# ldyken53/gaussian-splatting-wgpu

Hardware: AMD Instinct MI355X
Metric: frames/sec (higher is better)
Workload: dtype f32; 1 GPU; bicycle-like synthetic 6.1M gaussians @1920x1080; gaussians=6100000, width=1920, height=1080, tile_size=16, parallelism=single GPU, visible=2430918, processed=15909895, block_evaluated=6068168, sort_passes=1, depth_ordered_emission=True, tight_binning=True, blend_mode=fused, camera=64-step orbit, moved every frame

## Files before the change

### gaussian-splatting-wgpu_amd/csrc/gs_kernels.h

```cpp
#pragma once
#include "gs_device.h"

void gs_launch_repack(const void* d_aos, uint32_t n, const GsScene& s, hipStream_t st);
void gs_launch_ply_chunk(const void* d_raw, uint32_t m, uint32_t first, const GsPlyTable& t, const GsScene& s, hipStream_t st);
struct GsPreprocessLaunch {
    const void* func;
    uint32_t blocks;
    GsScene s; GsUniforms u; GsFrame f;
    void* gdata; uint32_t* counts; GsTightOut to;
    void* args[6];
};
void gs_preprocess_prepare(GsPreprocessLaunch& L, const GsScene& s, const GsUniforms& u, const GsFrame& f, void* gdata, uint32_t* counts,
                           bool tight, uint32_t* arena, uint32_t* rowptr, GsControl* ctl, uint32_t tight_nb = 0);
void gs_launch_preprocess(GsPreprocessLaunch& L, hipStream_t st);
void gs_launch_zero(void* p, uint64_t bytes, hipStream_t st);
uint32_t gs_scan_blocks(uint32_t n);
void gs_launch_scan(const uint32_t* counts, uint32_t n, uint32_t* offsets, unsigned long long* status, uint32_t* ticket, GsControl* ctl,
                    hipStream_t st);
uint64_t gs_emit_chunks(uint64_t capacity);
void gs_launch_emit_balanced(const void* gdata, const void* grec, const uint32_t* chunk_table, const GsFrame& f, uint32_t* keys, uint32_t* values,
                             GsControl* ctl, uint32_t grid, uint32_t hist_bits, uint32_t hist_passes, bool keys16, hipStream_t st);
void gs_launch_emit(const void* gdata, const uint32_t* counts, const uint32_t* offsets, const uint32_t* perm, const uint32_t* n_dev,
                    const GsFrame& f, uint32_t* keys, uint32_t* values, GsControl* ctl, hipStream_t st);
void gs_launch_ranges16(const uint16_t* tiles, const GsControl* ctl, uint32_t capacity, uint32_t T, uint32_t* ranges, uint32_t grid,
                        uint32_t* sticky, GsReport* rep, hipStream_t st);
void gs_launch_rebuild_keys(const uint16_t* tiles, const uint32_t* vals, const uint32_t* counts, uint32_t count, uint32_t n, uint32_t id_mask,
                            uint32_t* keys, hipStream_t st);
void gs_launch_ranges(const uint32_t* keys, const GsControl* ctl, uint32_t capacity, uint32_t T, uint32_t* ranges, uint32_t grid,
                      uint32_t* sticky, GsReport* rep, hipStream_t st);
uint32_t gs_sort_tiles(uint64_t capacity);
void gs_launch_sort(uint32_t* keysA, uint32_t* valsA, uint32_t* keysB, uint32_t* valsB, GsControl* ctl, uint32_t* tickets, uint32_t* hist,
                    const uint32_t* n_ptr, uint32_t capacity, uint32_t passes, uint32_t bits, uint32_t by_tile, uint32_t* status,
                    uint32_t grid, bool have_hist, const uint32_t* aux_table, uint32_t* aux_out, hipStream_t st, uint32_t** out_keys,
                    uint32_t** out_vals, bool keys16 = false);
int gs_launch_blend(const void* gdata, const uint32_t* values, const uint32_t* ranges, const GsFrame& f, uint32_t* rgba8, float* rgbf,
                    bool aux, float* alpha, float* depth, GsControl* ctl, uint32_t* tile_depth, bool exact, uint32_t ablation, bool masked, hipStream_t st, uint32_t* prof = nullptr,
                    uint32_t* prof_blocks = nullptr);
void gs_launch_debug_view(const uint32_t* ranges, const GsFrame& f, uint32_t view, uint32_t* rgba8, hipStream_t st);
void gs_launch_assemble(const void* slabs, void* image, uint32_t width, uint32_t height, const uint32_t* d_px_bounds, uint32_t n_slabs,
                        uint64_t slab_stride_px, hipStream_t st);
uint32_t gs_gsort_tiles(uint32_t n);
uint64_t gs_gsort_scratch_bytes(uint32_t n);
void gs_launch_gsort(const uint32_t* words, const uint32_t* aux_in, uint32_t n, void* scratch, void* grec, uint32_t* chunk_table, uint32_t chunk_cap,
                     uint32_t* tot_visible, uint32_t* tot_quantity, hipStream_t st);
uint32_t gs_rows_sort_tiles(uint64_t row_cap);
uint32_t gs_rows_chunks(uint64_t row_cap);
void gs_launch_rows(const uint32_t* arena, const void* grec, const uint32_t* chunk_table, uint32_t* rows_sorted, GsControl* ctl, uint32_t* sort_status, uint32_t row_cap,
                    uint32_t* M3, uint32_t* tileoff, uint32_t* rowtot, const GsFrame& f, uint32_t* values, uint32_t* ranges, uint32_t cus,
                    uint32_t* sticky, GsReport* rep, hipStream_t st, void (*mark)(void*, int), void* mark_arg);
void gs_launch_rows_rebuild_keys(const uint32_t* ranges, uint32_t T, const uint32_t* vals, const uint32_t* counts, uint32_t count, uint32_t n,
                                 uint32_t* keys, hipStream_t st);
void gs_launch_pick(const void* gdata, const uint32_t* values, const uint32_t* ranges, const GsFrame& f, uint32_t id_mask, const void* d_queries,
                    uint32_t n, void* d_results, uint32_t max_contrib, void* d_contrib, hipStream_t st);
```

### gaussian-splatting-wgpu_amd/csrc/gs_runtime.hip

```cpp
#include <hip/hip_runtime.h>

#include <algorithm>
#include <cmath>
#include <cstdarg>
#include <cstddef>
#include <cstdio>
#include <cstring>
#include <mutex>
#include <new>
#include <vector>

#include "../../include/gsplat/gs_abi.h"
#include "gs_kernels.h"
#include "gs_tight.h"

#define GS_EXPORT extern "C" __attribute__((visibility("default")))

static thread_local char g_err[512] = "";
static int32_t fail(int32_t code, const char* fmt, ...) {
    va_list ap;
    va_start(ap, fmt);
    vsnprintf(g_err, sizeof(g_err), fmt, ap);
    va_end(ap);
    return code;
// ... 336 lines not shown
    if (n) gs_launch_repack(d_aos, (uint32_t)n, c->scene, c->stream);
    HIP_TRY(hipGetLastError());
    HIP_TRY(hipStreamSynchronize(c->stream));
    return GS_OK;
}

static int32_t drop_shadows(gs_ctx* c) {
    for (gs_ctx* s : c->shadows) gs_destroy(s);
    c->shadows.clear();
    c->last = c;
    c->rr = 0;
    c->cap_hint = 0;
    c->row_hint = 0;
    return GS_OK;
}
GS_EXPORT int32_t gs_share_splats(gs_ctx* c, gs_ctx* owner) {
    if (!c || !owner || c == owner) return fail(GS_ERR_INVALID_ARGUMENT, "gs_share_splats: needs two distinct contexts");
    if (c->cfg.device != owner->cfg.device) return fail(GS_ERR_INVALID_ARGUMENT, "gs_share_splats: contexts are on different devices");
    if (!c->is_shadow) drop_shadows(c);
    if (!owner->scene_mem) return fail(GS_ERR_NO_SCENE, "gs_share_splats: the owner holds no splats");
    HIP_TRY(hipSetDevice(c->cfg.device));
    if (c->pending) { int32_t rc = wait_one(c); if (rc != GS_OK) return rc; }
    int32_t rc = alloc_per_gaussian(c, owner->n, c->cfg.max_intersections ? 0 : owner->capacity, owner->row_cap);
    if (rc != GS_OK) return rc;
    c->scene_mem = owner->scene_mem;
    c->scene_bytes = owner->scene_bytes;
    c->scene = owner->scene;
    c->scene_borrowed = true;
    HIP_TRY(hipStreamSynchronize(c->stream));
    return GS_OK;
}

GS_EXPORT int32_t gs_upload_splats_device(gs_ctx* c, const void* d_aos, uint64_t n) {
    if (!c || (!d_aos && n)) return fail(GS_ERR_INVALID_ARGUMENT, "gs_upload_splats_device: null argument");
    if (n >= (1ull << 31)) return fail(GS_ERR_INVALID_ARGUMENT, "gs_upload_splats: too many gaussians");
    HIP_TRY(hipSetDevice(c->cfg.device));
    drop_shadows(c);
    return upload_common(c, d_aos, n);
}

GS_EXPORT int32_t gs_upload_splats(gs_ctx* c, const void* aos, uint64_t n) {
    if (!c || (!aos && n)) return fail(GS_ERR_INVALID_ARGUMENT, "gs_upload_splats: null argument");
    if (n >= (1ull << 31)) return fail(GS_ERR_INVALID_ARGUMENT, "gs_upload_splats: too many gaussians");
    HIP_TRY(hipSetDevice(c->cfg.device));
    drop_shadows(c);
    void* d = nullptr;
    const size_t bytes = (size_t)n * GS_SPLAT_RECORD_BYTES;
    HIP_TRY(hipMalloc(&d, std::max<size_t>(bytes, 256)));
    if (bytes) {
        hipError_t e = hipMemcpy(d, aos, bytes, hipMemcpyHostToDevice);
        if (e != hipSuccess) { hipFree(d); return fail(GS_ERR_HIP, "upload memcpy: %s", hipGetErrorString(e)); }
    }
    int32_t rc = upload_common(c, d, n);
    hipFree(d);
    return rc;
}

static inline void mark(gs_ctx* c, int i) {
    if (!c->have_events) return;
    hipEventRecord(c->ev[c->frames % GS_EV_RING][i], c->stream);
    Roctx& r = roctx();
    if (r.push) {
        if (i > 0) r.pop();
        if (i < GS_STAGE_COUNT) r.push(kStageRange[i]);
    }
}

static void mark_cb(void* p, int i) { mark((gs_ctx*)p, i); }

static int32_t record_frame(gs_ctx* c, const GsUniforms& u, bool debug, void* ext_rgba8, bool tight) {
    const GsFrame& f = c->frame;
    hipStream_t st = c->stream;
    gs_launch_zero(c->ctl_mem, tight ? c->ctl_bytes_tight : c->ctl_bytes, st);
    c->h_ctl_valid = false;
    if (debug) HIP_TRY(hipMemsetAsync(c->gdata, 0, std::max<size_t>((size_t)c->n * 64, 256), st));
    mark(c, 0);
    gs_preprocess_prepare(c->pre, c->scene, u, f, c->gdata, c->counts, tight, c->arena, c->rowptr, c->ctl, c->tight_nb);
    gs_launch_preprocess(c->pre, st);
    mark(c, 1);
    const bool by_index = !tight && (debug || c->index_order);
    bool keys16 = false;
    if (tight) {
        gs_launch_gsort(c->counts, c->rowptr, c->n, c->gsort_scratch, c->grec, c->chunk_table, (uint32_t)gs_emit_chunks(std::max(c->capacity, c->row_cap)),
                        &c->ctl->num_visible, &c->ctl->num_slots, st);
        mark(c, 2);
        gs_launch_rows(c->arena, c->grec, c->chunk_table, c->rows_sorted, c->ctl, c->rows_status, (uint32_t)c->row_cap, c->M3, c->tileoff, c->rowtot, f, c->valsA,
                       c->ranges, c->grid_persist / 4u, c->sticky, c->h_rep, st, mark_cb, c);
        c->keysS = nullptr;
        c->valsS = c->valsA;
        mark(c, 4);
    } else if (by_index) {
        gs_launch_scan(c->counts, c->n, c->offsets, c->scan_status, &c->ctl->scan_ticket[0], c->ctl, st);
        mark(c, 2);
        gs_launch_emit(c->gdata, c->counts, c->offsets, nullptr, nullptr, f, c->keysA, c->valsA, c->ctl, st);
    } else {
        gs_launch_gsort(c->counts, nullptr, c->n, c->gsort_scratch, c->grec, c->chunk_table, (uint32_t)gs_emit_chunks(std::max(c->capacity, c->row_cap)),
                        &c->ctl->num_visible, &c->ctl->num_intersections, st);
        mark(c, 2);
        gs_launch_emit_balanced(c->gdata, c->grec, c->chunk_table, f, c->keysA, c->valsA, c->ctl, c->grid_persist * 2,
                                c->tile_bits, c->tile_passes, c->tile16, st);
        keys16 = c->tile16;
    }
    if (debug) {
        if (!c->keysU) {
            HIP_TRY(hipMalloc((void**)&c->keysU, (size_t)c->capacity * 4));
            HIP_TRY(hipMalloc((void**)&c->valsU, (size_t)c->capacity * 4));
        }
        HIP_TRY(hipMemcpyAsync(c->keysU, c->keysA, (size_t)c->capacity * 4, hipMemcpyDeviceToDevice, st));
        HIP_TRY(hipMemcpyAsync(c->valsU, c->valsA, (size_t)c->capacity * 4, hipMemcpyDeviceToDevice, st));
    }
    if (!tight) {
        mark(c, 3);
        if (by_index)
            gs_launch_sort(c->keysA, c->valsA, c->keysB, c->valsB, c->ctl, c->ctl->sort_ticket, &c->ctl->hist[0][0], &c->ctl->num_intersections,
                           (uint32_t)c->capacity, c->passes, 8, 0, c->sort_status, c->grid_persist, false, nullptr, nullptr, st, &c->keysS, &c->valsS);
        else
            gs_launch_sort(c->keysA, c->valsA, c->keysB, c->valsB, c->ctl, c->ctl->sort_ticket, &c->ctl->hist[0][0], &c->ctl->num_intersections,
                           (uint32_t)c->capacity, c->tile_passes, c->tile_bits, keys16 ? 0 : 1, c->sort_status, c->grid_persist, true,
                           nullptr, nullptr, st, &c->keysS, &c->valsS, keys16);
        mark(c, 4);
        if (keys16) gs_launch_ranges16((const uint16_t*)c->keysS, c->ctl, (uint32_t)c->capacity, c->T, c->ranges, c->grid_persist * 2, c->sticky, c->h_rep, st);
        else gs_launch_ranges(c->keysS, c->ctl, (uint32_t)c->capacity, c->T, c->ranges, c->grid_persist * 2, c->sticky, c->h_rep, st);
    }
    c->last_passes = tight ? 1u : (by_index ? c->passes : c->tile_passes);
    c->last_by_index = by_index;
    c->last_keys16 = keys16;
    c->last_tight = tight;
    mark(c, 5);
    uint32_t* target = ext_rgba8 ? (uint32_t*)ext_rgba8 : c->rgba8;
    if ((c->blend_ablation & 0x10000u) && !c->blend_prof) HIP_TRY(hipMalloc((void**)&c->blend_prof, (size_t)(1u << 20) * 16));
    const bool aux = (c->cfg.flags & GS_FLAG_AUX_OUTPUTS) != 0;
    const int walkers = gs_launch_blend(c->gdata, c->valsS, c->ranges, f, target, c->rgbf, aux, c->alpha, c->depth, c->ctl, c->tile_depth,
                                        (c->cfg.flags & GS_FLAG_EXACT_BLEND) != 0, c->blend_ablation & 0xFFFFu, tight, st,
                                        (c->blend_ablation & 0x10000u) ? c->blend_prof : nullptr, &c->blend_prof_blocks);
    if (walkers == -2) return fail(GS_ERR_INVALID_ARGUMENT, "blend: GS_FLAG_AUX_OUTPUTS without its alpha / depth planes");
    if (walkers < 0) return fail(GS_ERR_INVALID_ARGUMENT, "unsupported tile size %u", f.tile_size);
    c->blend_walkers = (uint32_t)walkers;
    mark(c, 6);
    if (c->debug_view) gs_launch_debug_view(c->ranges, f, c->debug_view, target, st);
    return GS_OK;
}

static void drop_graph(gs_ctx* c) {
    if (c->gexec) hipGraphExecDestroy(c->gexec);
    if (c->graph) hipGraphDestroy(c->graph);
    c->gexec = nullptr; c->graph = nullptr; c->pre_node = nullptr;
    c->graph_valid = false;
}

static int32_t enqueue_frame(gs_ctx* c, const GsUniforms& u, bool debug, void* ext_rgba8) {
    hipStream_t st = c->stream;
    if (c->emit_order == 2) {
        const uint64_t saved = c->passes > c->tile_passes ? c->passes - c->tile_passes : 0;
        c->index_order = !(c->have_frame && saved * (uint64_t)c->h_rep->num_intersections >= 1000000ull);
    } else {
        c->index_order = (c->emit_order == 1);
    }
    const bool tight = !debug && c->tile_cull && c->tight_ok && c->n < (1u << GS_ID_BITS);
    const bool graphable = c->use_graph && !debug && !c->have_events && !(c->blend_ablation & 0x10000u) && c->n;
    if (graphable) {
        if (!c->gexec || !c->graph_valid || c->gkey_index != c->index_order || c->gkey_tight != tight || c->gkey_ext != ext_rgba8 ||
            c->gkey_alpha != c->alpha || c->gkey_depth != c->depth) {
            if (c->gexec) HIP_TRY(hipStreamSynchronize(st));
            drop_graph(c);
            HIP_TRY(hipStreamBeginCapture(st, hipStreamCaptureModeRelaxed));
            const int32_t rc = record_frame(c, u, debug, ext_rgba8, tight);
            hipGraph_t g = nullptr;
            const hipError_t e = hipStreamEndCapture(st, &g);
            if (rc != GS_OK) { if (g) hipGraphDestroy(g); return rc; }
            if (e != hipSuccess || !g) return fail(GS_ERR_HIP, "frame graph capture: %s", hipGetErrorString(e));
            c->graph = g;
            HIP_TRY(hipGraphInstantiate(&c->gexec, g, nullptr, nullptr, 0));
            size_t nn = 0;
            HIP_TRY(hipGraphGetNodes(g, nullptr, &nn));
            std::vector<hipGraphNode_t> nodes(nn);
            HIP_TRY(hipGraphGetNodes(g, nodes.data(), &nn));
            uint32_t found = 0;
            for (hipGraphNode_t nd : nodes) {
                hipGraphNodeType ty;
                if (hipGraphNodeGetType(nd, &ty) != hipSuccess || ty != hipGraphNodeTypeKernel) continue;
// ... 796 lines not shown
```

### gaussian-splatting-wgpu_amd/csrc/k_gsort.hip

```cpp
#include "gs_device.h"

#define GC_ITEMS 8
#define GC_THREADS 256
#define GC (GC_THREADS * GC_ITEMS)
#define GBINS 1024
#define GS_EMIT_CHUNK_SHIFT 10
__device__ __forceinline__ uint64_t m_index(uint32_t b, uint32_t chunk, uint32_t NT) { return ((uint64_t)(b >> 3) * NT + chunk) * 8u + (b & 7u); }

__device__ __forceinline__ uint32_t sat32(unsigned long long v) { return v > 0xFFFFFFFFull ? 0xFFFFFFFFu : (uint32_t)v; }

__global__ __launch_bounds__(GC_THREADS) void gs_gsort_hist_kernel(const uint32_t* __restrict__ words, uint32_t n, uint2* __restrict__ M, uint32_t NT) {
    __shared__ uint32_t s_cnt[GBINS];
    __shared__ unsigned long long s_sum[GBINS];
    const uint32_t chunk = blockIdx.x, tid = threadIdx.x;
    for (uint32_t b = tid; b < GBINS; b += GC_THREADS) { s_cnt[b] = 0u; s_sum[b] = 0ull; }
    __syncthreads();
#pragma unroll
    for (int j = 0; j < GC_ITEMS; ++j) {
        const uint32_t k = chunk * GC + j * GC_THREADS + tid;
        if (k < n) {
            const uint32_t w = words[k];
            if (w & GS_COUNT_MASK) {
                const uint32_t b = w >> GS_COUNT_BITS;
                atomicAdd(&s_cnt[b], 1u);
                atomicAdd(&s_sum[b], (unsigned long long)(w & GS_COUNT_MASK));
            }
        }
    }
    __syncthreads();
#pragma unroll
    for (uint32_t i = 0; i < GBINS / GC_THREADS; ++i) {
        const uint32_t b = tid * (GBINS / GC_THREADS) + i;
        M[m_index(b, chunk, NT)] = make_uint2(s_cnt[b], sat32(s_sum[b]));
    }
}

struct GsPair { uint32_t x; unsigned long long y; };
__device__ __forceinline__ unsigned long long wave_incl_scan64(unsigned long long v, uint32_t lane) {
#pragma unroll
    for (int d = 1; d < 64; d <<= 1) {
        const uint32_t lo = __shfl_up((uint32_t)v, d, 64), hi = __shfl_up((uint32_t)(v >> 32), d, 64);
        if ((int)lane >= d) v += ((unsigned long long)hi << 32) | lo;
    }
    return v;
}
__device__ __forceinline__ GsPair block_excl2(GsPair v, uint32_t tid, GsPair* s_w , GsPair& total) {
    const uint32_t lane = tid & 63, w = tid >> 6;
    const uint32_t ix = wave_incl_scan(v.x, lane);
    const unsigned long long iy = wave_incl_scan64(v.y, lane);
    if (lane == 63) { s_w[w].x = ix; s_w[w].y = iy; }
    __syncthreads();
    GsPair base; base.x = 0u; base.y = 0ull;
    total.x = 0u; total.y = 0ull;
#pragma unroll
    for (int k = 0; k < GC_THREADS / 64; ++k) {
        const GsPair t = s_w[k];
        if (k < (int)w) { base.x += t.x; base.y += t.y; }
        total.x += t.x; total.y += t.y;
    }
    __syncthreads();
    GsPair r; r.x = base.x + ix - v.x; r.y = base.y + iy - v.y;
    return r;
}

#define GR_THREADS 1024
__device__ __forceinline__ void scan_stride8(uint32_t& x, unsigned long long& y, uint32_t lane) {
#pragma unroll
    for (int d = 8; d < 64; d <<= 1) {
        const uint32_t ox = __shfl_up(x, d, 64), lo = __shfl_up((uint32_t)y, d, 64), hi = __shfl_up((uint32_t)(y >> 32), d, 64);
        if ((int)lane >= d) { x += ox; y += ((unsigned long long)hi << 32) | lo; }
    }
}
__global__ __launch_bounds__(GR_THREADS) void gs_gsort_rowscan_kernel(uint2* __restrict__ M, uint32_t NT, uint32_t n, uint2* __restrict__ rowtot) {
    __shared__ uint32_t s_x[GR_THREADS / 64][8];
    __shared__ unsigned long long s_y[GR_THREADS / 64][8];
    const uint32_t nt = (n + GC - 1) / GC, tid = threadIdx.x, lane = tid & 63, w = tid >> 6, cl = tid >> 3, sub = tid & 7u;
    const uint32_t per = (nt + GR_THREADS / 8 - 1u) / (GR_THREADS / 8);
    const uint32_t c0 = cl * per < nt ? cl * per : nt, c1 = (cl + 1u) * per < nt ? (cl + 1u) * per : nt;
    uint2* row = M + (uint64_t)blockIdx.x * NT * 8u + sub;
    uint32_t ax = 0;
    unsigned long long ay = 0;
    for (uint32_t c = c0; c < c1; c += 8u) {
        uint2 v[8];
#pragma unroll
        for (int k = 0; k < 8; ++k) v[k] = (c + k < c1) ? row[(uint64_t)(c + k) * 8u] : make_uint2(0u, 0u);
#pragma unroll
        for (int k = 0; k < 8; ++k) { ax += v[k].x; ay += v[k].y; }
    }
    uint32_t ix = ax;
    unsigned long long iy = ay;
    scan_stride8(ix, iy, lane);
    if (lane >= 56u) { s_x[w][sub] = ix; s_y[w][sub] = iy; }
    __syncthreads();
    uint32_t rx = ix - ax, tx = 0;
    unsigned long long ry = iy - ay, ty = 0;
#pragma unroll
    for (uint32_t k = 0; k < GR_THREADS / 64; ++k) {
        const uint32_t vx = s_x[k][sub];
        const unsigned long long vy = s_y[k][sub];
        if (k < w) { rx += vx; ry += vy; }
        tx += vx; ty += vy;
    }
    for (uint32_t c = c0; c < c1; c += 8u) {
        uint2 v[8];
#pragma unroll
        for (int k = 0; k < 8; ++k) v[k] = (c + k < c1) ? row[(uint64_t)(c + k) * 8u] : make_uint2(0u, 0u);
#pragma unroll
        for (int k = 0; k < 8; ++k) {
            if (c + k < c1) row[(uint64_t)(c + k) * 8u] = make_uint2(rx, sat32(ry));
            rx += v[k].x; ry += v[k].y;
        }
    }
    if (tid < 8u) rowtot[blockIdx.x * 8u + sub] = make_uint2(tx, sat32(ty));
}

struct GsortShared {
    uint2 base[GBINS];
    unsigned short binstart[GBINS];
    union {
        unsigned short whist[GC_THREADS / 64][GBINS];
        uint32_t P[GC];
    } u;
    unsigned short id[GC];
    uint32_t word[GC], aux[GC];
    GsPair w2[GC_THREADS / 64];
    uint32_t wcnt[GC_THREADS / 64];
};
static_assert(sizeof(unsigned short) * (GC_THREADS / 64) * GBINS == sizeof(uint32_t) * GC, "the ranking counters and the prefix share their storage");

__global__ __launch_bounds__(GC_THREADS) void gs_gsort_scatter_kernel(const uint32_t* __restrict__ words, const uint32_t* __restrict__ aux_in, uint32_t n,
                                                                      const uint2* __restrict__ M, uint32_t NT, const uint2* __restrict__ rowtot,
                                                                      uint4* __restrict__ grec, uint32_t* __restrict__ chunk_table,
                                                                      uint32_t chunk_cap, uint32_t* __restrict__ tot_visible,
                                                                      uint32_t* __restrict__ tot_quantity) {
    __shared__ GsortShared S;
    const uint32_t chunk = blockIdx.x;
    const uint32_t tid = threadIdx.x, lane = tid & 63, w = tid >> 6;
    const unsigned long long lt_mask = (1ull << lane) - 1ull;
    constexpr uint32_t BPT = GBINS / GC_THREADS;

    uint32_t wv[GC_ITEMS], av[GC_ITEMS];
    const uint32_t e0 = chunk * GC + w * (64 * GC_ITEMS) + lane;
#pragma unroll
    for (int j = 0; j < GC_ITEMS; ++j) {
        const uint32_t k = e0 + j * 64;
        wv[j] = (k < n) ? words[k] : 0u;
        av[j] = (aux_in && k < n) ? aux_in[k] : 0u;
    }
    uint2 t[BPT], mm[BPT];
#pragma unroll
    for (uint32_t i = 0; i < BPT; ++i) { t[i] = rowtot[tid * BPT + i]; mm[i] = M[m_index(tid * BPT + i, chunk, NT)]; }

    {
        GsPair acc; acc.x = 0u; acc.y = 0ull;
#pragma unroll
        for (uint32_t i = 0; i < BPT; ++i) { acc.x += t[i].x; acc.y += t[i].y; }
        GsPair total;
        GsPair run = block_excl2(acc, tid, S.w2, total);
#pragma unroll
        for (uint32_t i = 0; i < BPT; ++i) {
            S.base[tid * BPT + i] = make_uint2(run.x + mm[i].x, sat32(run.y + mm[i].y));
            run.x += t[i].x; run.y += t[i].y;
        }
        if (chunk == 0 && tid == 0) { *tot_visible = total.x; *tot_quantity = sat32(total.y); }
    }
    for (uint32_t k = lane; k < GBINS; k += 64) S.u.whist[w][k] = 0;

    uint32_t wave_vis = 0;
#pragma unroll
    for (int j = 0; j < GC_ITEMS; ++j) {
        if (!(wv[j] & GS_COUNT_MASK)) wv[j] = 0u;
        wave_vis += (uint32_t)__popcll(__ballot(wv[j] != 0u));
    }
    if (lane == 0) S.wcnt[w] = wave_vis;
    __syncthreads();
    uint32_t cbase = 0, nc = 0;
#pragma unroll
    for (int k = 0; k < GC_THREADS / 64; ++k) { if (k < (int)w) cbase += S.wcnt[k]; nc += S.wcnt[k]; }
#pragma unroll
    for (int j = 0; j < GC_ITEMS; ++j) {
        const unsigned long long bal = __ballot(wv[j] != 0u);
        if (wv[j]) {
            const uint32_t p = cbase + (uint32_t)__popcll(bal & lt_mask);
            S.id[p] = (unsigned short)(w * (64 * GC_ITEMS) + j * 64 + lane);
            S.word[p] = wv[j];
            S.aux[p] = av[j];
        }
        cbase += (uint32_t)__popcll(bal);
    }
    for (uint32_t p = nc + tid; p < GC; p += GC_THREADS) S.word[p] = 0xFFFFFFFFu;
    __syncthreads();
    if (nc == 0) return;

    const uint32_t T = (nc + GC_THREADS - 1) / GC_THREADS;
    const uint32_t Q = T * 64;
    uint32_t gid[GC_ITEMS], wd[GC_ITEMS], ax[GC_ITEMS];
    uint32_t rank2[GC_ITEMS / 2];
#pragma unroll
    for (int j = 0; j < GC_ITEMS; ++j) {
        const uint32_t p = w * Q + j * 64 + lane;
        const bool in = (uint32_t)j < T;
        gid[j] = in ? (uint32_t)S.id[p] : 0u;
        wd[j] = in ? S.word[p] : 0xFFFFFFFFu;
        ax[j] = in ? S.aux[p] : 0u;
    }
#pragma unroll
    for (int j = 0; j < GC_ITEMS; ++j) {
        if ((uint32_t)j < T) {
            const uint32_t d = wd[j] >> GS_COUNT_BITS;
            uint32_t plo = 0xFFFFFFFFu, phi = 0xFFFFFFFFu;
#pragma unroll
            for (int b = 0; b < 10; ++b) {
                const uint32_t bit = (d >> b) & 1u;
                const unsigned long long bal = __ballot(bit != 0u);
                const uint32_t inv = bit - 1u;
                plo &= (uint32_t)bal ^ inv;
                phi &= (uint32_t)(bal >> 32) ^ inv;
            }
            const uint32_t below = __popc(plo & (uint32_t)lt_mask) + __popc(phi & (uint32_t)(lt_mask >> 32));
            const uint32_t cnt = __popc(plo) + __popc(phi);
            const uint32_t pre = S.u.whist[w][d];
            __builtin_amdgcn_fence(__ATOMIC_RELEASE, "wavefront");
            if (below == 0) S.u.whist[w][d] = (unsigned short)(pre + cnt);
            __builtin_amdgcn_fence(__ATOMIC_ACQUIRE, "wavefront");
            const uint32_t r = pre + below;
            if (j & 1) rank2[j >> 1] |= r << 16;
            else rank2[j >> 1] = r;
        }
    }
    __syncthreads();
    {
        uint32_t tot[BPT], acc = 0;
#pragma unroll
        for (uint32_t i = 0; i < BPT; ++i) {
            const uint32_t b = tid * BPT + i;
            uint32_t run = 0;
#pragma unroll
            for (int k = 0; k < GC_THREADS / 64; ++k) { const uint32_t c = S.u.whist[k][b]; S.u.whist[k][b] = (unsigned short)run; run += c; }
            tot[i] = run;
            acc += run;
        }
        GsPair total, in;
        in.x = acc; in.y = 0ull;
        const GsPair ex = block_excl2(in, tid, S.w2, total);
        uint32_t run = ex.x;
#pragma unroll
        for (uint32_t i = 0; i < BPT; ++i) { S.binstart[tid * BPT + i] = (unsigned short)run; run += tot[i]; }
    }
    __syncthreads();
    uint32_t mypos[GC_ITEMS];
#pragma unroll
    for (int j = 0; j < GC_ITEMS; ++j) {
        mypos[j] = 0xFFFFFFFFu;
        if ((uint32_t)j < T) {
            const uint32_t d = wd[j] >> GS_COUNT_BITS;
            const uint32_t r = (j & 1) ? (rank2[j >> 1] >> 16) : (rank2[j >> 1] & 0xFFFFu);
            mypos[j] = (uint32_t)S.binstart[d] + (uint32_t)S.u.whist[w][d] + r;
        }
    }
    __syncthreads();
#pragma unroll
    for (int j = 0; j < GC_ITEMS; ++j) {
        if ((uint32_t)j < T) {
            S.id[mypos[j]] = (unsigned short)gid[j];
            S.word[mypos[j]] = wd[j];
            S.aux[mypos[j]] = ax[j];
        }
    }
    __syncthreads();
    {
        uint32_t c[GC_ITEMS];
        unsigned long long acc = 0;
#pragma unroll
        for (int j = 0; j < GC_ITEMS; ++j) {
            const uint32_t p = tid * GC_ITEMS + j;
            const uint32_t x = (p < T * GC_THREADS) ? S.word[p] : 0xFFFFFFFFu;
            c[j] = x == 0xFFFFFFFFu ? 0u : (x & GS_COUNT_MASK);
            acc += c[j];
        }
        GsPair total, in;
        in.x = 0u; in.y = acc;
        const GsPair ex = block_excl2(in, tid, S.w2, total);
        unsigned long long run = ex.y;
#pragma unroll
        for (int j = 0; j < GC_ITEMS; ++j) { S.u.P[tid * GC_ITEMS + j] = sat32(run); run += c[j]; }
    }
    __syncthreads();
#pragma unroll
    for (int j = 0; j < GC_ITEMS; ++j) {
        const uint32_t pos = j * GC_THREADS + tid;
        if (pos >= nc) continue;
        const uint32_t x = S.word[pos];
        const uint32_t b = x >> GS_COUNT_BITS, first = S.binstart[b];
        const uint2 base = S.base[b];
        const uint32_t g = base.x + (pos - first);
        const unsigned long long off64 = (unsigned long long)base.y + (S.u.P[pos] - S.u.P[first]);
        const uint32_t off = sat32(off64);
        grec[g] = make_uint4(chunk * GC + (uint32_t)S.id[pos], x, off, S.aux[pos]);
        const uint32_t cnt = x & GS_COUNT_MASK;
        if (off != 0xFFFFFFFFu) {
            const unsigned long long lastq = (off64 + cnt - 1ull) >> GS_EMIT_CHUNK_SHIFT;
            const uint32_t last = lastq > 0xFFFFFFFFull ? 0xFFFFFFFFu : (uint32_t)lastq;
            for (uint32_t c = (uint32_t)((off64 + (1u << GS_EMIT_CHUNK_SHIFT) - 1ull) >> GS_EMIT_CHUNK_SHIFT); c <= last && c < chunk_cap; ++c) chunk_table[c] = g;
        }
    }
}

uint32_t gs_gsort_tiles(uint32_t n) { return (n + GC - 1) / GC; }
uint64_t gs_gsort_scratch_bytes(uint32_t n) { return ((uint64_t)GBINS * gs_gsort_tiles(n ? n : 1) + GBINS) * sizeof(uint2); }
void gs_launch_gsort(const uint32_t* words, const uint32_t* aux_in, uint32_t n, void* scratch, void* grec, uint32_t* chunk_table, uint32_t chunk_cap,
                     uint32_t* tot_visible, uint32_t* tot_quantity, hipStream_t st) {
    if (!n) return;
    const uint32_t NT = gs_gsort_tiles(n);
    uint2* M = (uint2*)scratch;
    uint2* rowtot = M + (uint64_t)GBINS * NT;
    hipLaunchKernelGGL(gs_gsort_hist_kernel, dim3(NT), dim3(GC_THREADS), 0, st, words, n, M, NT);
    hipLaunchKernelGGL(gs_gsort_rowscan_kernel, dim3(GBINS / 8), dim3(GR_THREADS), 0, st, M, NT, n, rowtot);
    hipLaunchKernelGGL(gs_gsort_scatter_kernel, dim3(NT), dim3(GC_THREADS), 0, st, words, aux_in, n, (const uint2*)M, NT, (const uint2*)rowtot,
                       (uint4*)grec, chunk_table, chunk_cap, tot_visible, tot_quantity);
}
```

Before: 1296 frames/s.

## Process multiple chunks per workgroup in gaussian depth sort with running bin bases

The histogram and scatter kernels of the gaussian depth-bin sort now each handle a run of consecutive chunks sized from the persistent grid, instead of one workgroup per chunk. Per-bin bases are carried forward across chunks inside the workgroup, and the next chunk's words are prefetched while the current one is processed. The histogram matrix shrinks to one column per run, which lightens the row scan. The scatter path also drops the separate compaction pass and ranks visible entries directly with ballots. The cost is less parallelism per launch and a serial dependence across chunks within each workgroup.

```diff
diff --git a/gaussian-splatting-wgpu_amd/csrc/gs_kernels.h b/gaussian-splatting-wgpu_amd/csrc/gs_kernels.h
--- a/gaussian-splatting-wgpu_amd/csrc/gs_kernels.h
+++ b/gaussian-splatting-wgpu_amd/csrc/gs_kernels.h
@@ -42,7 +42,7 @@
 uint32_t gs_gsort_tiles(uint32_t n);
 uint64_t gs_gsort_scratch_bytes(uint32_t n);
 void gs_launch_gsort(const uint32_t* words, const uint32_t* aux_in, uint32_t n, void* scratch, void* grec, uint32_t* chunk_table, uint32_t chunk_cap,
-                     uint32_t* tot_visible, uint32_t* tot_quantity, hipStream_t st);
+                     uint32_t* tot_visible, uint32_t* tot_quantity, uint32_t grid, hipStream_t st);
 uint32_t gs_rows_sort_tiles(uint64_t row_cap);
 uint32_t gs_rows_chunks(uint64_t row_cap);
 void gs_launch_rows(const uint32_t* arena, const void* grec, const uint32_t* chunk_table, uint32_t* rows_sorted, GsControl* ctl, uint32_t* sort_status, uint32_t row_cap,
diff --git a/gaussian-splatting-wgpu_amd/csrc/gs_runtime.hip b/gaussian-splatting-wgpu_amd/csrc/gs_runtime.hip
--- a/gaussian-splatting-wgpu_amd/csrc/gs_runtime.hip
+++ b/gaussian-splatting-wgpu_amd/csrc/gs_runtime.hip
@@ -442,7 +442,7 @@
     bool keys16 = false;
     if (tight) {
         gs_launch_gsort(c->counts, c->rowptr, c->n, c->gsort_scratch, c->grec, c->chunk_table, (uint32_t)gs_emit_chunks(std::max(c->capacity, c->row_cap)),
-                        &c->ctl->num_visible, &c->ctl->num_slots, st);
+                        &c->ctl->num_visible, &c->ctl->num_slots, c->grid_persist, st);
         mark(c, 2);
         gs_launch_rows(c->arena, c->grec, c->chunk_table, c->rows_sorted, c->ctl, c->rows_status, (uint32_t)c->row_cap, c->M3, c->tileoff, c->rowtot, f, c->valsA,
                        c->ranges, c->grid_persist / 4u, c->sticky, c->h_rep, st, mark_cb, c);
@@ -455,7 +455,7 @@
         gs_launch_emit(c->gdata, c->counts, c->offsets, nullptr, nullptr, f, c->keysA, c->valsA, c->ctl, st);
     } else {
         gs_launch_gsort(c->counts, nullptr, c->n, c->gsort_scratch, c->grec, c->chunk_table, (uint32_t)gs_emit_chunks(std::max(c->capacity, c->row_cap)),
-                        &c->ctl->num_visible, &c->ctl->num_intersections, st);
+                        &c->ctl->num_visible, &c->ctl->num_intersections, c->grid_persist, st);
         mark(c, 2);
         gs_launch_emit_balanced(c->gdata, c->grec, c->chunk_table, f, c->keysA, c->valsA, c->ctl, c->grid_persist * 2,
                                 c->tile_bits, c->tile_passes, c->tile16, st);
diff --git a/gaussian-splatting-wgpu_amd/csrc/k_gsort.hip b/gaussian-splatting-wgpu_amd/csrc/k_gsort.hip
--- a/gaussian-splatting-wgpu_amd/csrc/k_gsort.hip
+++ b/gaussian-splatting-wgpu_amd/csrc/k_gsort.hip
@@ -5,33 +5,51 @@
 #define GC (GC_THREADS * GC_ITEMS)
 #define GBINS 1024
 #define GS_EMIT_CHUNK_SHIFT 10
-__device__ __forceinline__ uint64_t m_index(uint32_t b, uint32_t chunk, uint32_t NT) { return ((uint64_t)(b >> 3) * NT + chunk) * 8u + (b & 7u); }
+#ifndef GS_GSORT_RUNS_Q
+#define GS_GSORT_RUNS_Q 4
+#endif
+__device__ __forceinline__ uint64_t m_index(uint32_t b, uint32_t col, uint32_t ncol) { return ((uint64_t)(b >> 3) * ncol + col) * 8u + (b & 7u); }
 
 __device__ __forceinline__ uint32_t sat32(unsigned long long v) { return v > 0xFFFFFFFFull ? 0xFFFFFFFFu : (uint32_t)v; }
 
-__global__ __launch_bounds__(GC_THREADS) void gs_gsort_hist_kernel(const uint32_t* __restrict__ words, uint32_t n, uint2* __restrict__ M, uint32_t NT) {
+__global__ __launch_bounds__(GC_THREADS) void gs_gsort_hist_kernel(const uint32_t* __restrict__ words, uint32_t n, uint2* __restrict__ M, uint32_t ncol,
+                                                                   uint32_t cpr, uint32_t NT) {
     __shared__ uint32_t s_cnt[GBINS];
     __shared__ unsigned long long s_sum[GBINS];
-    const uint32_t chunk = blockIdx.x, tid = threadIdx.x;
+    const uint32_t run = blockIdx.x, tid = threadIdx.x;
+    const uint32_t c0 = run * cpr, c1 = c0 + cpr < NT ? c0 + cpr : NT;
     for (uint32_t b = tid; b < GBINS; b += GC_THREADS) { s_cnt[b] = 0u; s_sum[b] = 0ull; }
-    __syncthreads();
+    uint32_t wv[GC_ITEMS];
 #pragma unroll
     for (int j = 0; j < GC_ITEMS; ++j) {
-        const uint32_t k = chunk * GC + j * GC_THREADS + tid;
-        if (k < n) {
-            const uint32_t w = words[k];
+        const uint32_t k = c0 * GC + j * GC_THREADS + tid;
+        wv[j] = (k < n) ? words[k] : 0u;
+    }
+    __syncthreads();
+    for (uint32_t c = c0; c < c1; ++c) {
+        uint32_t nx[GC_ITEMS];
+#pragma unroll
+        for (int j = 0; j < GC_ITEMS; ++j) {
+            const uint32_t k = (c + 1u) * GC + j * GC_THREADS + tid;
+            nx[j] = (c + 1u < c1 && k < n) ? words[k] : 0u;
+        }
+#pragma unroll
+        for (int j = 0; j < GC_ITEMS; ++j) {
+            const uint32_t w = wv[j];
             if (w & GS_COUNT_MASK) {
                 const uint32_t b = w >> GS_COUNT_BITS;
                 atomicAdd(&s_cnt[b], 1u);
                 atomicAdd(&s_sum[b], (unsigned long long)(w & GS_COUNT_MASK));
             }
         }
+#pragma unroll
+        for (int j = 0; j < GC_ITEMS; ++j) wv[j] = nx[j];
     }
     __syncthreads();
 #pragma unroll
     for (uint32_t i = 0; i < GBINS / GC_THREADS; ++i) {
         const uint32_t b = tid * (GBINS / GC_THREADS) + i;
-        M[m_index(b, chunk, NT)] = make_uint2(s_cnt[b], sat32(s_sum[b]));
+        M[m_index(b, run, ncol)] = make_uint2(s_cnt[b], sat32(s_sum[b]));
     }
 }
 
@@ -63,6 +81,24 @@
     return r;
 }
 
+template <typename A>
+__device__ __forceinline__ A block_excl_u32(uint32_t v, uint32_t tid, uint32_t* s_w , A& total) {
+    const uint32_t lane = tid & 63, w = tid >> 6;
+    const uint32_t iv = wave_incl_scan(v, lane);
+    if (lane == 63) s_w[w] = iv;
+    __syncthreads();
+    A base = 0;
+    total = 0;
+#pragma unroll
+    for (int k = 0; k < GC_THREADS / 64; ++k) {
+        const uint32_t t = s_w[k];
+        if (k < (int)w) base += t;
+        total += t;
+    }
+    __syncthreads();
+    return base + (iv - v);
+}
+
 #define GR_THREADS 1024
 __device__ __forceinline__ void scan_stride8(uint32_t& x, unsigned long long& y, uint32_t lane) {
 #pragma unroll
@@ -71,13 +107,13 @@
         if ((int)lane >= d) { x += ox; y += ((unsigned long long)hi << 32) | lo; }
     }
 }
-__global__ __launch_bounds__(GR_THREADS) void gs_gsort_rowscan_kernel(uint2* __restrict__ M, uint32_t NT, uint32_t n, uint2* __restrict__ rowtot) {
+__global__ __launch_bounds__(GR_THREADS) void gs_gsort_rowscan_kernel(uint2* __restrict__ M, uint32_t ncol, uint2* __restrict__ rowtot) {
     __shared__ uint32_t s_x[GR_THREADS / 64][8];
     __shared__ unsigned long long s_y[GR_THREADS / 64][8];
-    const uint32_t nt = (n + GC - 1) / GC, tid = threadIdx.x, lane = tid & 63, w = tid >> 6, cl = tid >> 3, sub = tid & 7u;
+    const uint32_t nt = ncol, tid = threadIdx.x, lane = tid & 63, w = tid >> 6, cl = tid >> 3, sub = tid & 7u;
     const uint32_t per = (nt + GR_THREADS / 8 - 1u) / (GR_THREADS / 8);
     const uint32_t c0 = cl * per < nt ? cl * per : nt, c1 = (cl + 1u) * per < nt ? (cl + 1u) * per : nt;
-    uint2* row = M + (uint64_t)blockIdx.x * NT * 8u + sub;
+    uint2* row = M + (uint64_t)blockIdx.x * ncol * 8u + sub;
     uint32_t ax = 0;
     unsigned long long ay = 0;
     for (uint32_t c = c0; c < c1; c += 8u) {
@@ -114,44 +150,59 @@
     if (tid < 8u) rowtot[blockIdx.x * 8u + sub] = make_uint2(tx, sat32(ty));
 }
 
-struct GsortShared {
+struct alignas(16) GsortShared {
     uint2 base[GBINS];
     unsigned short binstart[GBINS];
     union {
         unsigned short whist[GC_THREADS / 64][GBINS];
         uint32_t P[GC];
+        uint4 zero[GC / 4];
     } u;
     unsigned short id[GC];
     uint32_t word[GC], aux[GC];
     GsPair w2[GC_THREADS / 64];
-    uint32_t wcnt[GC_THREADS / 64];
+    uint32_t w1[GC_THREADS / 64];
+    uint32_t ptot;
 };
 static_assert(sizeof(unsigned short) * (GC_THREADS / 64) * GBINS == sizeof(uint32_t) * GC, "the ranking counters and the prefix share their storage");
+static_assert(sizeof(GsortShared) <= 40 * 1024, "four workgroups per CU");
 
 __global__ __launch_bounds__(GC_THREADS) void gs_gsort_scatter_kernel(const uint32_t* __restrict__ words, const uint32_t* __restrict__ aux_in, uint32_t n,
-                                                                      const uint2* __restrict__ M, uint32_t NT, const uint2* __restrict__ rowtot,
-                                                                      uint4* __restrict__ grec, uint32_t* __restrict__ chunk_table,
-                                                                      uint32_t chunk_cap, uint32_t* __restrict__ tot_visible,
-                                                                      uint32_t* __restrict__ tot_quantity) {
+                                                                      const uint2* __restrict__ M, uint32_t ncol, uint32_t cpr, uint32_t NT,
+                                                                      const uint2* __restrict__ rowtot, uint4* __restrict__ grec,
+                                                                      uint32_t* __restrict__ chunk_table, uint32_t chunk_cap,
+                                                                      uint32_t* __restrict__ tot_visible, uint32_t* __restrict__ tot_quantity) {
     __shared__ GsortShared S;
-    const uint32_t chunk = blockIdx.x;
+    const uint32_t run_id = blockIdx.x;
+    const uint32_t chunk0 = run_id * cpr, chunk1 = chunk0 + cpr < NT ? chunk0 + cpr : NT;
     const uint32_t tid = threadIdx.x, lane = tid & 63, w = tid >> 6;
     const unsigned long long lt_mask = (1ull << lane) - 1ull;
     constexpr uint32_t BPT = GBINS / GC_THREADS;
 
-    uint32_t wv[GC_ITEMS], av[GC_ITEMS];
-    const uint32_t e0 = chunk * GC + w * (64 * GC_ITEMS) + lane;
-#pragma unroll
-    for (int j = 0; j < GC_ITEMS; ++j) {
-        const uint32_t k = e0 + j * 64;
-        wv[j] = (k < n) ? words[k] : 0u;
-        av[j] = (aux_in && k < n) ? aux_in[k] : 0u;
-    }
-    uint2 t[BPT], mm[BPT];
-#pragma unroll
-    for (uint32_t i = 0; i < BPT; ++i) { t[i] = rowtot[tid * BPT + i]; mm[i] = M[m_index(tid * BPT + i, chunk, NT)]; }
-
+    uint32_t nwv[GC_ITEMS], nav[GC_ITEMS];
+    const uint32_t whole = n / GC;
+    auto load_chunk = [&](uint32_t c) {
+        const uint32_t k0 = c * GC + w * (64 * GC_ITEMS) + lane;
+        if (c < whole) {
+#pragma unroll
+            for (int j = 0; j < GC_ITEMS; ++j) nwv[j] = words[k0 + j * 64];
+#pragma unroll
+            for (int j = 0; j < GC_ITEMS; ++j) nav[j] = aux_in ? aux_in[k0 + j * 64] : 0u;
+        } else {
+#pragma unroll
+            for (int j = 0; j < GC_ITEMS; ++j) {
+                const uint32_t k = k0 + j * 64;
+                nwv[j] = (k < n) ? words[k] : 0u;
+                nav[j] = (aux_in && k < n) ? aux_in[k] : 0u;
+            }
+        }
+    };
+    load_chunk(chunk0);
     {
+        uint2 t[BPT], mm[BPT];
+#pragma unroll
+        for (uint32_t i = 0; i < BPT; ++i) { t[i] = rowtot[tid * BPT + i]; mm[i] = M[m_index(tid * BPT + i, run_id, ncol)]; }
+
         GsPair acc; acc.x = 0u; acc.y = 0ull;
 #pragma unroll
         for (uint32_t i = 0; i < BPT; ++i) { acc.x += t[i].x; acc.y += t[i].y; }
@@ -162,146 +213,130 @@
             S.base[tid * BPT + i] = make_uint2(run.x + mm[i].x, sat32(run.y + mm[i].y));
             run.x += t[i].x; run.y += t[i].y;
         }
-        if (chunk == 0 && tid == 0) { *tot_visible = total.x; *tot_quantity = sat32(total.y); }
-    }
-    for (uint32_t k = lane; k < GBINS; k += 64) S.u.whist[w][k] = 0;
-
-    uint32_t wave_vis = 0;
-#pragma unroll
-    for (int j = 0; j < GC_ITEMS; ++j) {
-        if (!(wv[j] & GS_COUNT_MASK)) wv[j] = 0u;
-        wave_vis += (uint32_t)__popcll(__ballot(wv[j] != 0u));
-    }
-    if (lane == 0) S.wcnt[w] = wave_vis;
-    __syncthreads();
-    uint32_t cbase = 0, nc = 0;
-#pragma unroll
-    for (int k = 0; k < GC_THREADS / 64; ++k) { if (k < (int)w) cbase += S.wcnt[k]; nc += S.wcnt[k]; }
-#pragma unroll
-    for (int j = 0; j < GC_ITEMS; ++j) {
-        const unsigned long long bal = __ballot(wv[j] != 0u);
-        if (wv[j]) {
-            const uint32_t p = cbase + (uint32_t)__popcll(bal & lt_mask);
-            S.id[p] = (unsigned short)(w * (64 * GC_ITEMS) + j * 64 + lane);
-            S.word[p] = wv[j];
-            S.aux[p] = av[j];
-        }
-        cbase += (uint32_t)__popcll(bal);
-    }
-    for (uint32_t p = nc + tid; p < GC; p += GC_THREADS) S.word[p] = 0xFFFFFFFFu;
-    __syncthreads();
-    if (nc == 0) return;
-
-    const uint32_t T = (nc + GC_THREADS - 1) / GC_THREADS;
-    const uint32_t Q = T * 64;
-    uint32_t gid[GC_ITEMS], wd[GC_ITEMS], ax[GC_ITEMS];
-    uint32_t rank2[GC_ITEMS / 2];
-#pragma unroll
-    for (int j = 0; j < GC_ITEMS; ++j) {
-        const uint32_t p = w * Q + j * 64 + lane;
-        const bool in = (uint32_t)j < T;
-        gid[j] = in ? (uint32_t)S.id[p] : 0u;
-        wd[j] = in ? S.word[p] : 0xFFFFFFFFu;
-        ax[j] = in ? S.aux[p] : 0u;
-    }
-#pragma unroll
-    for (int j = 0; j < GC_ITEMS; ++j) {
-        if ((uint32_t)j < T) {
-            const uint32_t d = wd[j] >> GS_COUNT_BITS;
-            uint32_t plo = 0xFFFFFFFFu, phi = 0xFFFFFFFFu;
-#pragma unroll
-            for (int b = 0; b < 10; ++b) {
-                const uint32_t bit = (d >> b) & 1u;
-                const unsigned long long bal = __ballot(bit != 0u);
-                const uint32_t inv = bit - 1u;
-                plo &= (uint32_t)bal ^ inv;
-                phi &= (uint32_t)(bal >> 32) ^ inv;
-            }
-            const uint32_t below = __popc(plo & (uint32_t)lt_mask) + __popc(phi & (uint32_t)(lt_mask >> 32));
-            const uint32_t cnt = __popc(plo) + __popc(phi);
-            const uint32_t pre = S.u.whist[w][d];
-            __builtin_amdgcn_fence(__ATOMIC_RELEASE, "wavefront");
-            if (below == 0) S.u.whist[w][d] = (unsigned short)(pre + cnt);
-            __builtin_amdgcn_fence(__ATOMIC_ACQUIRE, "wavefront");
-            const uint32_t r = pre + below;
+        if (run_id == 0 && tid == 0) { *tot_visible = total.x; *tot_quantity = sat32(total.y); }
+    }
+
+    for (uint32_t chunk = chunk0; chunk < chunk1; ++chunk) {
+        uint32_t wv[GC_ITEMS], av[GC_ITEMS];
+#pragma unroll
+        for (int j = 0; j < GC_ITEMS; ++j) { wv[j] = nwv[j]; av[j] = nav[j]; }
+        if (chunk + 1u < chunk1) load_chunk(chunk + 1u);
+        {
+            S.u.zero[w * (GBINS / 8) + lane] = make_uint4(0u, 0u, 0u, 0u);
+            S.u.zero[w * (GBINS / 8) + 64 + lane] = make_uint4(0u, 0u, 0u, 0u);
+        }
+        uint32_t rank2[GC_ITEMS / 2];
+#pragma unroll
+        for (int j = 0; j < GC_ITEMS; ++j) {
+            if (!(wv[j] & GS_COUNT_MASK)) wv[j] = 0u;
+            const unsigned long long vis = __ballot(wv[j] != 0u);
+            uint32_t r = 0;
+            if (vis) {
+                const uint32_t d = wv[j] >> GS_COUNT_BITS;
+                uint32_t plo = (uint32_t)vis, phi = (uint32_t)(vis >> 32);
+#pragma unroll
+                for (int b = 0; b < 10; ++b) {
+                    const uint32_t bit = (d >> b) & 1u;
+                    const unsigned long long bal = __ballot(bit != 0u);
+                    const uint32_t inv = bit - 1u;
+                    plo &= (uint32_t)bal ^ inv;
+                    phi &= (uint32_t)(bal >> 32) ^ inv;
+                }
+                const uint32_t below = __popc(plo & (uint32_t)lt_mask) + __popc(phi & (uint32_t)(lt_mask >> 32));
+                const uint32_t cnt = __popc(plo) + __popc(phi);
+                const uint32_t pre = S.u.whist[w][d];
+                __builtin_amdgcn_fence(__ATOMIC_RELEASE, "wavefront");
+                if (wv[j] && below == 0) S.u.whist[w][d] = (unsigned short)(pre + cnt);
+                __builtin_amdgcn_fence(__ATOMIC_ACQUIRE, "wavefront");
+                r = pre + below;
+            }
             if (j & 1) rank2[j >> 1] |= r << 16;
             else rank2[j >> 1] = r;
         }
-    }
-    __syncthreads();
-    {
-        uint32_t tot[BPT], acc = 0;
-#pragma unroll
-        for (uint32_t i = 0; i < BPT; ++i) {
-            const uint32_t b = tid * BPT + i;
-            uint32_t run = 0;
-#pragma unroll
-            for (int k = 0; k < GC_THREADS / 64; ++k) { const uint32_t c = S.u.whist[k][b]; S.u.whist[k][b] = (unsigned short)run; run += c; }
-            tot[i] = run;
-            acc += run;
-        }
-        GsPair total, in;
-        in.x = acc; in.y = 0ull;
-        const GsPair ex = block_excl2(in, tid, S.w2, total);
-        uint32_t run = ex.x;
-#pragma unroll
-        for (uint32_t i = 0; i < BPT; ++i) { S.binstart[tid * BPT + i] = (unsigned short)run; run += tot[i]; }
-    }
-    __syncthreads();
-    uint32_t mypos[GC_ITEMS];
-#pragma unroll
-    for (int j = 0; j < GC_ITEMS; ++j) {
-        mypos[j] = 0xFFFFFFFFu;
-        if ((uint32_t)j < T) {
-            const uint32_t d = wd[j] >> GS_COUNT_BITS;
-            const uint32_t r = (j & 1) ? (rank2[j >> 1] >> 16) : (rank2[j >> 1] & 0xFFFFu);
-            mypos[j] = (uint32_t)S.binstart[d] + (uint32_t)S.u.whist[w][d] + r;
-        }
-    }
-    __syncthreads();
-#pragma unroll
-    for (int j = 0; j < GC_ITEMS; ++j) {
-        if ((uint32_t)j < T) {
-            S.id[mypos[j]] = (unsigned short)gid[j];
-            S.word[mypos[j]] = wd[j];
-            S.aux[mypos[j]] = ax[j];
-        }
-    }
-    __syncthreads();
-    {
-        uint32_t c[GC_ITEMS];
-        unsigned long long acc = 0;
-#pragma unroll
-        for (int j = 0; j < GC_ITEMS; ++j) {
-            const uint32_t p = tid * GC_ITEMS + j;
-            const uint32_t x = (p < T * GC_THREADS) ? S.word[p] : 0xFFFFFFFFu;
-            c[j] = x == 0xFFFFFFFFu ? 0u : (x & GS_COUNT_MASK);
-            acc += c[j];
-        }
-        GsPair total, in;
-        in.x = 0u; in.y = acc;
-        const GsPair ex = block_excl2(in, tid, S.w2, total);
-        unsigned long long run = ex.y;
-#pragma unroll
-        for (int j = 0; j < GC_ITEMS; ++j) { S.u.P[tid * GC_ITEMS + j] = sat32(run); run += c[j]; }
-    }
-    __syncthreads();
-#pragma unroll
-    for (int j = 0; j < GC_ITEMS; ++j) {
-        const uint32_t pos = j * GC_THREADS + tid;
-        if (pos >= nc) continue;
-        const uint32_t x = S.word[pos];
-        const uint32_t b = x >> GS_COUNT_BITS, first = S.binstart[b];
-        const uint2 base = S.base[b];
-        const uint32_t g = base.x + (pos - first);
-        const unsigned long long off64 = (unsigned long long)base.y + (S.u.P[pos] - S.u.P[first]);
-        const uint32_t off = sat32(off64);
-        grec[g] = make_uint4(chunk * GC + (uint32_t)S.id[pos], x, off, S.aux[pos]);
-        const uint32_t cnt = x & GS_COUNT_MASK;
-        if (off != 0xFFFFFFFFu) {
-            const unsigned long long lastq = (off64 + cnt - 1ull) >> GS_EMIT_CHUNK_SHIFT;
-            const uint32_t last = lastq > 0xFFFFFFFFull ? 0xFFFFFFFFu : (uint32_t)lastq;
-            for (uint32_t c = (uint32_t)((off64 + (1u << GS_EMIT_CHUNK_SHIFT) - 1ull) >> GS_EMIT_CHUNK_SHIFT); c <= last && c < chunk_cap; ++c) chunk_table[c] = g;
+        __syncthreads();
+        uint32_t nc;
+        {
+            uint32_t tot[BPT], acc = 0;
+#pragma unroll
+            for (uint32_t i = 0; i < BPT; ++i) {
+                const uint32_t b = tid * BPT + i;
+                uint32_t run = 0;
+#pragma unroll
+                for (int k = 0; k < GC_THREADS / 64; ++k) { const uint32_t c = S.u.whist[k][b]; S.u.whist[k][b] = (unsigned short)run; run += c; }
+                tot[i] = run;
+                acc += run;
+            }
+            uint32_t run = block_excl_u32<uint32_t>(acc, tid, S.w1, nc);
+#pragma unroll
+            for (uint32_t i = 0; i < BPT; ++i) { S.binstart[tid * BPT + i] = (unsigned short)run; run += tot[i]; }
+        }
+        if (nc == 0) continue;
+        __syncthreads();
+#pragma unroll
+        for (int j = 0; j < GC_ITEMS; ++j) {
+            if (wv[j]) {
+                const uint32_t d = wv[j] >> GS_COUNT_BITS;
+                const uint32_t r = (j & 1) ? (rank2[j >> 1] >> 16) : (rank2[j >> 1] & 0xFFFFu);
+                const uint32_t pos = (uint32_t)S.binstart[d] + (uint32_t)S.u.whist[w][d] + r;
+                S.id[pos] = (unsigned short)(w * (64 * GC_ITEMS) + j * 64 + lane);
+                S.word[pos] = wv[j];
+                S.aux[pos] = av[j];
+            }
+        }
+        __syncthreads();
+        {
+            uint32_t c[GC_ITEMS], acc = 0;
+#pragma unroll
+            for (int j = 0; j < GC_ITEMS; ++j) {
+                const uint32_t p = tid * GC_ITEMS + j;
+                c[j] = (p < nc) ? (S.word[p] & GS_COUNT_MASK) : 0u;
+                acc += c[j];
+            }
+            unsigned long long total;
+            unsigned long long run = block_excl_u32<unsigned long long>(acc, tid, S.w1, total);
+#pragma unroll
+            for (int j = 0; j < GC_ITEMS; ++j) { S.u.P[tid * GC_ITEMS + j] = sat32(run); run += c[j]; }
+            if (tid == 0) S.ptot = sat32(total);
+        }
+        __syncthreads();
+#pragma unroll
+        for (int j = 0; j < GC_ITEMS; ++j) {
+            const uint32_t pos = j * GC_THREADS + tid;
+            if (pos >= nc) continue;
+            const uint32_t x = S.word[pos];
+            const uint32_t b = x >> GS_COUNT_BITS, first = S.binstart[b];
+            const uint2 base = S.base[b];
+            const uint32_t g = base.x + (pos - first);
+            const unsigned long long off64 = (unsigned long long)base.y + (S.u.P[pos] - S.u.P[first]);
+            const uint32_t off = sat32(off64);
+            grec[g] = make_uint4(chunk * GC + (uint32_t)S.id[pos], x, off, S.aux[pos]);
+            const uint32_t cnt = x & GS_COUNT_MASK;
+            if (off != 0xFFFFFFFFu) {
+                const unsigned long long lastq = (off64 + cnt - 1ull) >> GS_EMIT_CHUNK_SHIFT;
+                const uint32_t last = lastq > 0xFFFFFFFFull ? 0xFFFFFFFFu : (uint32_t)lastq;
+                for (uint32_t c = (uint32_t)((off64 + (1u << GS_EMIT_CHUNK_SHIFT) - 1ull) >> GS_EMIT_CHUNK_SHIFT); c <= last && c < chunk_cap; ++c) chunk_table[c] = g;
+            }
+        }
+        if (chunk + 1u < chunk1) {
+            uint32_t dx[BPT], py[BPT + 1];
+            uint32_t s = S.binstart[tid * BPT];
+            py[0] = s < GC ? S.u.P[s] : S.ptot;
+#pragma unroll
+            for (uint32_t i = 0; i < BPT; ++i) {
+                const uint32_t b = tid * BPT + i;
+                const uint32_t e = (b + 1u < GBINS) ? (uint32_t)S.binstart[b + 1u] : nc;
+                dx[i] = e - s;
+                py[i + 1] = e < GC ? S.u.P[e] : S.ptot;
+                s = e;
+            }
+            __syncthreads();
+#pragma unroll
+            for (uint32_t i = 0; i < BPT; ++i) {
+                uint2 v = S.base[tid * BPT + i];
+                v.x += dx[i];
+                v.y = py[i + 1] == 0xFFFFFFFFu ? 0xFFFFFFFFu : sat32((unsigned long long)v.y + (py[i + 1] - py[i]));
+                S.base[tid * BPT + i] = v;
+            }
         }
     }
 }
@@ -309,13 +344,17 @@
 uint32_t gs_gsort_tiles(uint32_t n) { return (n + GC - 1) / GC; }
 uint64_t gs_gsort_scratch_bytes(uint32_t n) { return ((uint64_t)GBINS * gs_gsort_tiles(n ? n : 1) + GBINS) * sizeof(uint2); }
 void gs_launch_gsort(const uint32_t* words, const uint32_t* aux_in, uint32_t n, void* scratch, void* grec, uint32_t* chunk_table, uint32_t chunk_cap,
-                     uint32_t* tot_visible, uint32_t* tot_quantity, hipStream_t st) {
+                     uint32_t* tot_visible, uint32_t* tot_quantity, uint32_t grid, hipStream_t st) {
     if (!n) return;
     const uint32_t NT = gs_gsort_tiles(n);
+    uint64_t want = (uint64_t)grid * GS_GSORT_RUNS_Q / 4u;
+    if (!want) want = 1;
+    const uint32_t cpr = (uint32_t)((NT + want - 1) / want);
+    const uint32_t G = (NT + cpr - 1) / cpr;
     uint2* M = (uint2*)scratch;
-    uint2* rowtot = M + (uint64_t)GBINS * NT;
-    hipLaunchKernelGGL(gs_gsort_hist_kernel, dim3(NT), dim3(GC_THREADS), 0, st, words, n, M, NT);
-    hipLaunchKernelGGL(gs_gsort_rowscan_kernel, dim3(GBINS / 8), dim3(GR_THREADS), 0, st, M, NT, n, rowtot);
-    hipLaunchKernelGGL(gs_gsort_scatter_kernel, dim3(NT), dim3(GC_THREADS), 0, st, words, aux_in, n, (const uint2*)M, NT, (const uint2*)rowtot,
+    uint2* rowtot = M + (uint64_t)GBINS * G;
+    hipLaunchKernelGGL(gs_gsort_hist_kernel, dim3(G), dim3(GC_THREADS), 0, st, words, n, M, G, cpr, NT);
+    hipLaunchKernelGGL(gs_gsort_rowscan_kernel, dim3(GBINS / 8), dim3(GR_THREADS), 0, st, M, G, rowtot);
+    hipLaunchKernelGGL(gs_gsort_scatter_kernel, dim3(G), dim3(GC_THREADS), 0, st, words, aux_in, n, (const uint2*)M, G, cpr, NT, (const uint2*)rowtot,
                        (uint4*)grec, chunk_table, chunk_cap, tot_visible, tot_quantity);
 }
```

Result: faster. 1332 frames/s, median of 6 (+2.8%).
